# stevenczwu/SAMBLE

Hardware: NVIDIA B200
Metric: clouds/sec SAMBLE seg fwd (N=2048) (higher is better)
Workload: dtype f32

## Files before the change

samble_b200/csrc/knn_tc.cu:

```cuda
#include <cuda_bf16.h>

#include "common.cuh"
#include "tc_common.cuh"

namespace samble {

constexpr int kTcRows = 128;
constexpr int kTcTile = 128;
constexpr int kTcStages = 5;
constexpr int kTcStagesA = 10;
constexpr int kExt = 4096;
constexpr int kTcCap = 120;
constexpr int kTcListLd = 128;
constexpr int kTcListSm = 129;
constexpr int kTcThreads = 192;

static size_t tc_smem_bytes(int nkt, bool pass_b) {
  return (size_t)(pass_b ? 2 : 1) * nkt * 16384 + (size_t)(pass_b ? kTcStages : kTcStagesA) * 16384
         + 3 * kExt  + (pass_b ? (size_t)kTcRows * kTcListSm * 4 : 0) + 1024 + 256;
}

__device__ __forceinline__ float knn_margin(float aa, float bbmax) {
  const float s = sqrtf(aa * bbmax);
  return (3.0517578e-05f + 0.00012207031f) * s + 3.0517578e-05f * (aa + bbmax);
}

__device__ __forceinline__ float knn_margin_coarse(float aa, float bbmax) {
  const float s = sqrtf(aa * bbmax);
  return (0.0078125f + 3.0517578e-05f + 0.00012207031f) * s + 3.0517578e-05f * (aa + bbmax);
}

__device__ __forceinline__ uint32_t knn_pack(float delta, int j) { return (__float_as_uint(delta) & 0xffff0000u) | (uint32_t)j; }
__device__ __forceinline__ float knn_delta_lo(uint32_t w) { return __uint_as_float(w & 0xffff0000u); }
__device__ __forceinline__ float knn_delta_hi(float lo) { return lo * 1.0079f; }

__device__ __forceinline__ void sort64(float (&v)[64]) {
#pragma unroll
  for (int ls = 1; ls <= 6; ++ls) {
#pragma unroll
    for (int lt = ls - 1; lt >= 0; --lt) {
      const int size = 1 << ls, stride = 1 << lt;
#pragma unroll
      for (int t = 0; t < 32; ++t) {
        const int lo = 2 * t - (t & (stride - 1));
        const int hi = lo + stride;
        const bool up = (lo & size) == 0;
        const float a = v[lo], b = v[hi];
        v[lo] = up ? fminf(a, b) : fmaxf(a, b);
        v[hi] = up ? fmaxf(a, b) : fminf(a, b);
      }
    }
  }
}

template <bool PASS_B, int CS, bool PROF = false>
__global__ void __cluster_dims__(CS, 1, 1) __launch_bounds__(kTcThreads, 1)
    knn_tc_kernel(const __grid_constant__ CUtensorMap map_a_hi, const __grid_constant__ CUtensorMap map_a_lo,
                  const __grid_constant__ CUtensorMap map_b_hi, const __grid_constant__ CUtensorMap map_b_lo,
                  const float* __restrict__ anorm, const float* __restrict__ bext, const unsigned* __restrict__ bbmax_bits,
                  int Nq, int Nr, int Cp, int k, float* __restrict__ thr, uint32_t* __restrict__ cand_out,
                  int* __restrict__ cnt_out, int dbg, long long* __restrict__ prof_out) {
  long long* const prof = PROF ? prof_out : nullptr;
  extern __shared__ uint8_t smem_raw[];
  uint8_t* base = tc::smem_align1024(smem_raw);
  const int nkt = (Cp + 63) / 64;
  constexpr int kPlanes = PASS_B ? 2 : 1;
  constexpr int kStages = PASS_B ? kTcStages : kTcStagesA;
  uint8_t* sA = base;
  uint8_t* sB = sA + (size_t)kPlanes * nkt * 16384;
  uint8_t* sAx = sB + (size_t)kStages * 16384;
  uint8_t* sBx = sAx + kExt;
  uint8_t* tail = sBx + 2 * kExt;
  uint32_t* cand = reinterpret_cast<uint32_t*>(tail);
  uint64_t* bars = reinterpret_cast<uint64_t*>(tail + (PASS_B ? kTcRows * kTcListSm * 4 : 0));
  uint64_t* full = bars;
  uint64_t* empty = bars + kStages;
  uint64_t* tfull = bars + 2 * kStages;
  uint64_t* tempty = tfull + 2;
  uint64_t* afull = tempty + 2;
  uint32_t* tmem_slot = reinterpret_cast<uint32_t*>(afull + 1);

  const int tid = threadIdx.x, warp = tid >> 5, lane = tid & 31;
  const int b = blockIdx.y, q0 = blockIdx.x * kTcRows;
  const int ntiles = (Nr + kTcTile - 1) / kTcTile;
  const uint32_t crank = CS > 1 ? tc::cluster_ctarank() : 0u;
  constexpr uint16_t kMask = (uint16_t)((1u << CS) - 1u);

  for (int p = tid; p < 256; p += kTcThreads) {
    const int row = p >> 1, ch = p & 1;
    *reinterpret_cast<uint4*>(sAx + tc::nosw_offset(row, ch, 128)) = ch == 0 ? make_uint4(0x3f803f80u, 0x00003f80u, 0u, 0u) : make_uint4(0u, 0u, 0u, 0u);
  }
  tc::fence_proxy_async();
  if (tid == 0) {
    for (int s = 0; s < kStages; ++s) {
      tc::mbar_init(&full[s], 1);
      tc::mbar_init(&empty[s], CS);
    }
    for (int a = 0; a < 2; ++a) {
      tc::mbar_init(&tfull[a], 1);
      tc::mbar_init(&tempty[a], 128);
    }
    tc::mbar_init(afull, 1);
    tc::mbar_init_fence();
  }
  if (warp == 0) tc::tmem_alloc(tmem_slot, 256);
  tc::tc_fence_before();
  __syncthreads();
  if (CS > 1) tc::cluster_sync();
  tc::tc_fence_after();
  const uint32_t tmem = *tmem_slot;

  if (warp == 5) {
    if (tc::elect_one()) {
      tc::tma_prefetch_desc(&map_a_hi);
      tc::tma_prefetch_desc(&map_b_hi);
      tc::tma_prefetch_desc(&map_b_lo);
      tc::mbar_arrive_expect_tx(afull, (uint32_t)(kPlanes * nkt) * 16384u);
      for (int kt = 0; kt < nkt; ++kt) {
        tc::tma_load_3d(sA + (size_t)kt * 16384, &map_a_hi, afull, kt * 64, q0, b);
        if (PASS_B) tc::tma_load_3d(sA + (size_t)(nkt + kt) * 16384, &map_a_lo, afull, kt * 64, q0, b);
      }
      const float* ext_g = bext + (size_t)b * ntiles * (kExt / 4);
      int s = 0, ph = 0;
      uint32_t seq = 0;
      long long w_empty = 0;
      const long long p_t0 = PROF ? clock64() : 0;
      for (int t = 0; t < ntiles; ++t) {
        for (int g = 0; g < kPlanes * nkt; ++g, ++seq) {
          const int kt = PASS_B ? g >> 1 : g;
          const long long p_t = (PROF && prof) ? clock64() : 0;
          tc::mbar_wait(&empty[s], ph ^ 1);
          if (PROF && prof) w_empty += clock64() - p_t;
          if (g == 0) {
            if (t >= 2) tc::mbar_wait(&tfull[t & 1], ((t - 2) >> 1) & 1);
            tc::mbar_arrive_expect_tx(&full[s], 16384u + kExt);
            tc::bulk_load_1d(sBx + (size_t)(t & 1) * kExt, ext_g + (size_t)t * (kExt / 4), kExt, &full[s]);
          } else {
            tc::mbar_arrive_expect_tx(&full[s], 16384u);
          }
          const CUtensorMap* mp = (PASS_B && (g & 1)) ? &map_b_lo : &map_b_hi;
          if (CS == 1)
            tc::tma_load_3d(sB + (size_t)s * 16384, mp, &full[s], kt * 64, t * kTcTile, b);
          else if (seq % CS == crank)
            tc::tma_load_3d_multicast(sB + (size_t)s * 16384, mp, &full[s], kt * 64, t * kTcTile, b, kMask);
          if (++s == kStages) { s = 0; ph ^= 1; }
        }
      }
      if (PROF && prof) {
        long long* o = prof + 8 * (blockIdx.y * gridDim.x + blockIdx.x);
        o[5] = clock64() - p_t0, o[6] = w_empty;
      }
    }
    __syncwarp();
  } else if (warp == 4) {
    if (tc::elect_one()) {
      const uint32_t idesc = tc::instr_desc(1, kTcRows, kTcTile);
      const uint64_t axd = tc::smem_desc_nosw(tc::smem_u32(sAx), 128);
      long long w_full = 0, w_tempty = 0, w_a = 0, w_issue = 0;
      const long long m_t0 = PROF ? clock64() : 0;
      tc::mbar_wait(afull, 0);
      if (PROF && prof) w_a = clock64() - m_t0;
      int s = 0, ph = 0;
      for (int t = 0; t < ntiles; ++t) {
        const int acc = t & 1;
        long long m_t = (PROF && prof) ? clock64() : 0;
        tc::mbar_wait(&tempty[acc], ((t >> 1) & 1) ^ 1);
        if (PROF && prof) w_tempty += clock64() - m_t;
        tc::tc_fence_after();
        for (int g = 0; g < kPlanes * nkt; ++g) {
          const int kt = PASS_B ? g >> 1 : g;
          m_t = (PROF && prof) ? clock64() : 0;
          tc::mbar_wait(&full[s], ph);
          if (PROF && prof) w_full += clock64() - m_t;
          tc::tc_fence_after();
          const long long i_t = (PROF && prof) ? clock64() : 0;
          const uint64_t ah = tc::smem_desc_sw128(tc::smem_u32(sA + (size_t)kt * 16384));
          const uint64_t al = tc::smem_desc_sw128(tc::smem_u32(sA + (size_t)(nkt + kt) * 16384));
          const uint64_t bd = tc::smem_desc_sw128(tc::smem_u32(sB + (size_t)s * 16384));
          if (dbg & 1) {
          } else if (!PASS_B || (g & 1) == 0) {
#pragma unroll
            for (int k16 = 0; k16 < 4; ++k16) tc::mma_bf16(tmem + acc * kTcTile, ah + 2 * k16, bd + 2 * k16, idesc, (g | k16) != 0);
            if (PASS_B) {
#pragma unroll
              for (int k16 = 0; k16 < 4; ++k16) tc::mma_bf16(tmem + acc * kTcTile, al + 2 * k16, bd + 2 * k16, idesc, 1);
            }
          } else {
#pragma unroll
            for (int k16 = 0; k16 < 4; ++k16) tc::mma_bf16(tmem + acc * kTcTile, ah + 2 * k16, bd + 2 * k16, idesc, 1);
          }
          if (PROF && prof) w_issue += clock64() - i_t;
          if (g == kPlanes * nkt - 1) {
            if (!(dbg & 1)) tc::mma_bf16(tmem + acc * kTcTile, axd, tc::smem_desc_nosw(tc::smem_u32(sBx + (size_t)(t & 1) * kExt), 128), idesc, 1);
          }
          if (CS == 1) tc::mma_commit(&empty[s]);
          else tc::mma_commit_multicast(&empty[s], kMask);
          if (++s == kStages) { s = 0; ph ^= 1; }
        }
        tc::mma_commit(&tfull[acc]);
      }
      if (PROF && prof) {
        long long* o = prof + 8 * (blockIdx.y * gridDim.x + blockIdx.x);
        o[0] = clock64() - m_t0, o[1] = w_full, o[2] = w_tempty, o[3] = w_a, o[7] = w_issue;
      }
    }
    __syncwarp();
  } else {
    const int row = warp * 32 + lane;
    const int q = q0 + row;
    const uint32_t lane_base = (uint32_t)(warp * 32) << 16;
    float gmax[64];
    float my_thr = 0.f;
    const uint32_t lbeg = tc::smem_u32(cand + row * kTcListSm);
    uint32_t lptr = lbeg;
    if (!PASS_B) {
#pragma unroll
      for (int i = 0; i < 64; ++i) gmax[i] = -INFINITY;
    } else {
      my_thr = q < Nq ? thr[(size_t)b * Nq + q] : INFINITY;
    }
    long long w_tfull = 0;
    for (int t = 0; t < ntiles; ++t) {
      const int acc = t & 1;
      const long long e_t = (PROF && prof) ? clock64() : 0;
      tc::mbar_wait(&tfull[acc], (t >> 1) & 1);
      if (PROF && prof) w_tfull += clock64() - e_t;
      tc::tc_fence_after();
      if (!(dbg & 2))
#pragma unroll
      for (int c0 = 0; c0 < kTcTile; c0 += 64) {
        float v[64];
        tc::tmem_ld64(tmem + lane_base + acc * kTcTile + c0, v);
        if (!PASS_B) {
#pragma unroll
          for (int i = 0; i < 64; ++i) gmax[i] = fmaxf(gmax[i], v[i]);
        } else {
          const int jbase = t * kTcTile + c0;
#pragma unroll
          for (int i = 0; i < 64; ++i) {
            const float delta = v[i] - my_thr;
            asm volatile("st.shared.u32 [%0], %1;" ::"r"(lptr), "r"(knn_pack(delta, jbase + i)) : "memory");
            lptr += delta >= 0.f ? 4u : 0u;
            if ((i & 7) == 7) lptr = min(lptr, lbeg + 4u * kTcCap);
          }
        }
      }
      tc::tc_fence_before();
      tc::mbar_arrive(&tempty[acc]);
    }
    if (PROF && prof && tid == 0) prof[8 * (blockIdx.y * gridDim.x + blockIdx.x) + 4] = w_tfull;
    if (!PASS_B) {
      if (q < Nq) {
        sort64(gmax);
        float kth = INFINITY;
#pragma unroll
        for (int i = 32; i < 64; ++i) kth = fminf(kth, i >= 64 - k ? gmax[i] : INFINITY);
        const float aa = anorm[(size_t)b * Nq + q];
        const float bbm = __uint_as_float(bbmax_bits[b]);
        const float e = knn_margin(aa, bbm), ea = knn_margin_coarse(aa, bbm);
        thr[(size_t)b * Nq + q] = fminf(kth - 0.5f * (ea + e), 0.5f * (aa - e));
      }
    } else if (q < Nq) {
      cnt_out[(size_t)b * Nq + q] = (int)(min(lptr, lbeg + 4u * kTcCap) - lbeg) >> 2;
    }
  }

  if (PASS_B) {
    __syncthreads();
    for (int row = warp; row < kTcRows; row += kTcThreads / 32) {
      const int q = q0 + row;
      if (q >= Nq) break;
#pragma unroll
      for (int u = 0; u < 4; ++u)
        cand_out[((size_t)b * Nq + q) * kTcListLd + u * 32 + lane] = cand[row * kTcListSm + u * 32 + lane];
    }
  }
  tc::tc_fence_before();
  __syncthreads();
  if (CS > 1) tc::cluster_sync();
  if (warp == 0) tc::tmem_dealloc(tmem, 256);
}

template <class I>
__device__ __forceinline__ void knn_exact_row(const float* __restrict__ arow, float aa, const float* __restrict__ B_g,
                                              const float* __restrict__ bnorm_g, int Nr, int Cp, int k, int lane,
                                              I* __restrict__ idx_row, float* __restrict__ dist_row, bool ordered) {
  const float4* ar = reinterpret_cast<const float4*>(arow);
  LaneTopK top;
  top.init(lane, k);
  for (int j0 = 0; j0 < Nr; j0 += 128) {
    float acc[4] = {0.f, 0.f, 0.f, 0.f};
    const float4* br[4];
#pragma unroll
    for (int u = 0; u < 4; ++u) br[u] = reinterpret_cast<const float4*>(B_g + (size_t)min(j0 + 32 * u + lane, Nr - 1) * Cp);
#pragma unroll 2
    for (int c4 = 0; c4 < Cp / 4; ++c4) {
      const float4 a4 = __ldg(ar + c4);
#pragma unroll
      for (int u = 0; u < 4; ++u) {
        const float4 b4 = __ldg(br[u] + c4);
        acc[u] = fmaf(a4.x, b4.x, acc[u]);
        acc[u] = fmaf(a4.y, b4.y, acc[u]);
        acc[u] = fmaf(a4.z, b4.z, acc[u]);
        acc[u] = fmaf(a4.w, b4.w, acc[u]);
      }
    }
#pragma unroll
    for (int u = 0; u < 4; ++u) {
      const int j = j0 + 32 * u + lane;
      const bool have = j < Nr;
      const float d2 = __fmaf_rn(-2.f, acc[u], __fadd_rn(aa, __ldg(bnorm_g + min(j, Nr - 1))));
      top.offer(dist_bits(d2), j, have);
    }
  }
  const int pos = ordered ? top.rank() : lane;
  if (top.active) {
    idx_row[pos] = (I)top.i;
    if (dist_row) dist_row[pos] = -sqrtf(__uint_as_float(top.d));
  }
}

template <class I>
__global__ void __launch_bounds__(256) knn_rerank_kernel(const float* __restrict__ an, const float* __restrict__ anorm,
                                                         const float* __restrict__ bn, const float* __restrict__ bnorm,
                                                         const uint32_t* __restrict__ cand,
                                                         const int* __restrict__ cnt_in, int Nq, int Nr, int Cp, int k,
                                                         I* __restrict__ idx_out, float* __restrict__ dist_out,
                                                         int* __restrict__ row_flags) {
  const int warp = threadIdx.x >> 5, lane = threadIdx.x & 31;
  const int b = blockIdx.y, q = blockIdx.x * 8 + warp;
  if (q >= Nq) return;
  const size_t rowi = (size_t)b * Nq + q;
  const int cnt = cnt_in[rowi];
  const float aa = anorm[rowi];
  const float4* ar = reinterpret_cast<const float4*>(an + rowi * Cp);
  const float* B_g = bn + (size_t)b * Nr * Cp;
  const float* bnorm_g = bnorm + (size_t)b * Nr;
  if (cnt >= kTcCap) {
    knn_exact_row<I>(an + rowi * Cp, aa, B_g, bnorm_g, Nr, Cp, k, lane, idx_out + rowi * k, dist_out ? dist_out + rowi * k : nullptr, true);
    return;
  }
  LaneTopK top;
  top.init(lane, k);
  for (int r = 0; r < cnt; r += 32) {
    const int e = r + lane;
    const bool have = e < cnt;
    const int j = have ? (int)(cand[rowi * kTcListLd + e] & 0xffffu) : 0;
    const float4* br = reinterpret_cast<const float4*>(B_g + (size_t)j * Cp);
    float acc = 0.f;
#pragma unroll 4
    for (int c4 = 0; c4 < Cp / 4; ++c4) {
      const float4 a4 = __ldg(ar + c4);
      const float4 b4 = __ldg(br + c4);
      acc = fmaf(a4.x, b4.x, acc);
      acc = fmaf(a4.y, b4.y, acc);
      acc = fmaf(a4.z, b4.z, acc);
      acc = fmaf(a4.w, b4.w, acc);
    }
    const float d2 = __fmaf_rn(-2.f, acc, __fadd_rn(aa, __ldg(bnorm_g + j)));
    const unsigned db = dist_bits(d2);
    if (r == 0 && cnt >= k) {
      top.fill(db, j, have && lane < k);
      top.offer(db, j, have && lane >= k);
    } else {
      top.offer(db, j, have);
    }
  }
  const int rk = top.rank();
  if (top.active) {
    const long long o = (long long)rowi * k + rk;
    idx_out[o] = (I)top.i;
    if (dist_out) dist_out[o] = -sqrtf(__uint_as_float(top.d));
  }
}

template <int NPL, class I>
__device__ __forceinline__ void select_classify(const uint32_t* __restrict__ list, int cnt, int k, float aa, float e,
                                                float thr_row, int lane, I* __restrict__ idx_row,
                                                unsigned short* __restrict__ amb, int& n_in, int& n_amb) {
  constexpr int kN = 32 * NPL;
  uint32_t w[NPL], x[NPL];
#pragma unroll
  for (int u = 0; u < NPL; ++u) {
    const int t = u * 32 + lane;
    w[u] = t < cnt ? __ldg(list + t) : 0u;
    x[u] = ~w[u];
  }
#pragma unroll
  for (int size = 2; size <= kN; size <<= 1) {
#pragma unroll
    for (int stride = size >> 1; stride >= 1; stride >>= 1) {
      if (stride >= 32) {
        const int du = stride >> 5;
#pragma unroll
        for (int u = 0; u < NPL; ++u) {
          if ((u & du) == 0) {
            const bool up = ((u * 32) & size) == 0;
            const uint32_t lo = min(x[u], x[u | du]), hi = max(x[u], x[u | du]);
            x[u] = up ? lo : hi;
            x[u | du] = up ? hi : lo;
          }
        }
      } else {
#pragma unroll
        for (int u = 0; u < NPL; ++u) {
          const uint32_t other = __shfl_xor_sync(kFull, x[u], stride);
          const bool up = ((u * 32 + lane) & size) == 0;
          const bool lower = (lane & stride) == 0;
          x[u] = (lower == up) ? min(x[u], other) : max(x[u], other);
        }
      }
    }
  }
  uint32_t xk = 0xffffffffu, xk1 = 0xffffffffu;
#pragma unroll
  for (int u = 0; u < NPL; ++u) {
    const uint32_t a0 = __shfl_sync(kFull, x[u], (k - 1) & 31);
    const uint32_t a1 = __shfl_sync(kFull, x[u], k & 31);
    if (((k - 1) >> 5) == u) xk = a0;
    if ((k >> 5) == u) xk1 = a1;
  }
  const float dk = knn_delta_lo(~xk);
  const float dk1 = cnt > k ? knn_delta_lo(~xk1) : -INFINITY;
  const float n0 = (0.5f * (aa - e) - thr_row) * 0.999f;
  const bool in_ok = knn_delta_hi(dk1) < n0 || cnt == k;
  const float in_thr = knn_delta_hi(dk1) + e;
  const float out_thr = dk - e;
  const unsigned lt = (1u << lane) - 1u;
#pragma unroll
  for (int u = 0; u < NPL; ++u) {
    const bool have = u * 32 + lane < cnt;
    const float dlo = knn_delta_lo(w[u]), dhi = knn_delta_hi(dlo);
    const int j = (int)(w[u] & 0xffffu);
    const bool is_in = have && in_ok && dlo > in_thr;
    const bool is_out = have && dhi < out_thr && dhi < n0;
    const bool is_amb = have && !is_in && !is_out;
    const unsigned m_in = __ballot_sync(kFull, is_in), m_amb = __ballot_sync(kFull, is_amb);
    if (is_in) idx_row[n_in + __popc(m_in & lt)] = (I)j;
    if (is_amb) amb[n_amb + __popc(m_amb & lt)] = (unsigned short)j;
    n_in += __popc(m_in);
    n_amb += __popc(m_amb);
  }
}

constexpr int kSelBatch = 4;
constexpr int kSelRowLd = 132;

template <class I>
__global__ void __launch_bounds__(256, 5) knn_select_kernel(const float* __restrict__ an, const float* __restrict__ anorm,
                                                         const float* __restrict__ bn, const float* __restrict__ bnorm,
                                                         const unsigned* __restrict__ bbmax_bits,
                                                         const uint32_t* __restrict__ cand,
                                                         const float* __restrict__ thr_in, const int* __restrict__ cnt_in,
                                                         int Nq, int Nr, int Cp, int k, I* __restrict__ idx_out,
                                                         int* __restrict__ row_flags) {
  __shared__ unsigned short amb[8][128];
  __shared__ __align__(16) float s_arow[8][128];
  __shared__ __align__(16) float s_rows[8][kSelBatch * kSelRowLd];
  __shared__ unsigned long long s_keys[8][128];
  const int warp = threadIdx.x >> 5, lane = threadIdx.x & 31;
  const int b = blockIdx.y, q = blockIdx.x * 8 + warp;
  if (q >= Nq) return;
  const size_t rowi = (size_t)b * Nq + q;
  const int cnt = cnt_in[rowi];
  const float aa = anorm[rowi];
  if (cnt >= kTcCap) {
    knn_exact_row<I>(an + rowi * Cp, aa, bn + (size_t)b * Nr * Cp, bnorm + (size_t)b * Nr, Nr, Cp, k, lane, idx_out + rowi * k, nullptr, false);
    return;
  }
  const float e = knn_margin(aa, __uint_as_float(bbmax_bits[b])) * 1.001f;
  int n_in = 0, n_amb = 0;
  const uint32_t* list = cand + rowi * kTcListLd;
  const float thr_row = __ldg(thr_in + rowi);
  if (cnt <= 32)
    select_classify<1, I>(list, cnt, k, aa, e, thr_row, lane, idx_out + rowi * k, amb[warp], n_in, n_amb);
  else if (cnt <= 64)
    select_classify<2, I>(list, cnt, k, aa, e, thr_row, lane, idx_out + rowi * k, amb[warp], n_in, n_amb);
  else
    select_classify<4, I>(list, cnt, k, aa, e, thr_row, lane, idx_out + rowi * k, amb[warp], n_in, n_amb);
  const int need = k - n_in;
  if (need <= 0) return;
  if (n_amb < need) {
    __syncwarp();
    knn_exact_row<I>(an + rowi * Cp, aa, bn + (size_t)b * Nr * Cp, bnorm + (size_t)b * Nr, Nr, Cp, k, lane, idx_out + rowi * k, nullptr, false);
    return;
  }
  __syncwarp();
  const int nch = Cp >> 2;
  const float4* ar = reinterpret_cast<const float4*>(an + rowi * Cp);
  const float* B_g = bn + (size_t)b * Nr * Cp;
  const float* bnorm_g = bnorm + (size_t)b * Nr;
  if (lane < nch) reinterpret_cast<float4*>(s_arow[warp])[lane] = __ldg(ar + lane);
  for (int r = 0; r < n_amb; r += kSelBatch) {
    const int nb = min(kSelBatch, n_amb - r);
    float4 tmp[kSelBatch];
#pragma unroll
    for (int u = 0; u < kSelBatch; ++u)
      if (u < nb && lane < nch) tmp[u] = __ldg(reinterpret_cast<const float4*>(B_g + (size_t)amb[warp][r + u] * Cp) + lane);
#pragma unroll
    for (int u = 0; u < kSelBatch; ++u)
      if (u < nb && lane < nch) reinterpret_cast<float4*>(s_rows[warp] + u * kSelRowLd)[lane] = tmp[u];
    __syncwarp();
    if (lane < nb) {
      const int j = (int)amb[warp][r + lane];
      const float4* br = reinterpret_cast<const float4*>(s_rows[warp] + lane * kSelRowLd);
      const float4* aq = reinterpret_cast<const float4*>(s_arow[warp]);
      float acc = 0.f;
#pragma unroll 4
      for (int c4 = 0; c4 < nch; ++c4) {
        const float4 a4 = aq[c4];
        const float4 b4 = br[c4];
        acc = fmaf(a4.x, b4.x, acc);
        acc = fmaf(a4.y, b4.y, acc);
        acc = fmaf(a4.z, b4.z, acc);
        acc = fmaf(a4.w, b4.w, acc);
      }
      const float d2 = __fmaf_rn(-2.f, acc, __fadd_rn(aa, __ldg(bnorm_g + j)));
      s_keys[warp][r + lane] = ((unsigned long long)dist_bits(d2) << 32) | (unsigned)j;
    }
    __syncwarp();
  }
  for (int t = lane; t < n_amb; t += 32) {
    const unsigned long long mine = s_keys[warp][t];
    int rank = 0;
    for (int u = 0; u < n_amb; ++u) rank += s_keys[warp][u] < mine ? 1 : 0;
    if (rank < need) idx_out[rowi * k + n_in + rank] = (I)(unsigned)(mine & 0xffffffffu);
  }
}

int g_knn_tc_debug = 0;
int g_knn_cluster = -1;
long long* g_knn_prof = nullptr;

size_t knn_tc_ext_floats(int B, int Nr);
bool knn_tc_eligible(int Nq, int Nr, int C, int k) {
  const int Cp = (int)align_up(C, 32);
  return C >= 4 && Cp <= 128 && k <= 32 && Nr <= 65535 && Nr >= k;
}

size_t knn_tc_workspace_bytes(int B, int Nq, int Nr) {
  return align_up((size_t)B * Nq * kTcListLd * sizeof(uint32_t), 256) + align_up((size_t)B * Nq * sizeof(int), 256) +
         align_up(knn_tc_ext_floats(B, Nr) * sizeof(float), 256);
}
size_t knn_tc_ext_floats(int B, int Nr) { return (size_t)B * ceil_div(Nr, kTcTile) * (kExt / 4); }

template <class I>
int launch_knn_tc(const float* an, const float* anorm, const float* bn, const float* bnorm, const __nv_bfloat16* a_hi,
                  const __nv_bfloat16* a_lo, const __nv_bfloat16* b_hi, const __nv_bfloat16* b_lo, const float* bext,
                  const unsigned* bbmax, int B, int Nq, int Nr, int Cp, int k, float* thr, uint32_t* cand, int* cnt, bool ordered,
                  I* idx, float* dist, int* row_flags, cudaStream_t st) {
  const int nkb = (Cp + 63) / 64;
  alignas(64) CUtensorMap map_a, map_al, map_b, map_bl;
  if (int e = make_tile_map(&map_a, a_hi, Cp, Cp, Nq, B, kTcRows, 2)) return e;
  if (int e = make_tile_map(&map_al, a_lo, Cp, Cp, Nq, B, kTcRows, 2)) return e;
  if (int e = make_tile_map(&map_b, b_hi, Cp, Cp, Nr, B, kTcTile, 2)) return e;
  if (int e = make_tile_map(&map_bl, b_lo, Cp, Cp, Nr, B, kTcTile, 2)) return e;
  dim3 grid(ceil_div(Nq, kTcRows), B);
  const int cs = g_knn_cluster > 0 ? g_knn_cluster : 1;
  {
    size_t smem = tc_smem_bytes(nkb, false);
    auto kern = cs == 2 ? knn_tc_kernel<false, 2> : (cs == 4 ? knn_tc_kernel<false, 4> : (g_knn_prof ? knn_tc_kernel<false, 1, true> : knn_tc_kernel<false, 1>));
    if (cudaFuncSetAttribute(kern, cudaFuncAttributeMaxDynamicSharedMemorySize, (int)smem) != cudaSuccess)
      return check_launch("knn_tc pass A smem attribute");
    SAMBLE_PRE(st);
    kern<<<grid, kTcThreads, smem, st>>>(map_a, map_al, map_b, map_bl, anorm, bext, bbmax, Nq, Nr, Cp, k, thr, cand, cnt, g_knn_tc_debug, g_knn_prof);
    SAMBLE_LAUNCHED("knn_tc_threshold_kernel");
  }
  {
    size_t smem = tc_smem_bytes(nkb, true);
    auto kern = cs == 2 ? knn_tc_kernel<true, 2> : (cs == 4 ? knn_tc_kernel<true, 4> : (g_knn_prof ? knn_tc_kernel<true, 1, true> : knn_tc_kernel<true, 1>));
    if (cudaFuncSetAttribute(kern, cudaFuncAttributeMaxDynamicSharedMemorySize, (int)smem) != cudaSuccess)
      return check_launch("knn_tc pass B smem attribute");
    SAMBLE_PRE(st);
    kern<<<grid, kTcThreads, smem, st>>>(map_a, map_al, map_b, map_bl, anorm, bext, bbmax, Nq, Nr, Cp, k, thr, cand, cnt, g_knn_tc_debug, g_knn_prof);
    SAMBLE_LAUNCHED("knn_tc_collect_kernel");
  }
  SAMBLE_PRE(st);
  if (ordered) {
    knn_rerank_kernel<I><<<dim3(ceil_div(Nq, 8), B), 256, 0, st>>>(an, anorm, bn, bnorm, cand, cnt, Nq, Nr, Cp, k, idx, dist, row_flags);
    SAMBLE_LAUNCHED("knn_rerank_kernel");
  } else {
    knn_select_kernel<I><<<dim3(ceil_div(Nq, 8), B), 256, 0, st>>>(an, anorm, bn, bnorm, bbmax, cand, thr, cnt, Nq, Nr, Cp, k, idx, row_flags);
    SAMBLE_LAUNCHED("knn_select_kernel");
  }
  return SAMBLE_OK;
}

template int launch_knn_tc<int>(const float*, const float*, const float*, const float*, const __nv_bfloat16*, const __nv_bfloat16*,
                                const __nv_bfloat16*, const __nv_bfloat16*, const float*, const unsigned*, int, int, int, int, int,
                                float*, uint32_t*, int*, bool, int*, float*, int*, cudaStream_t);
template int launch_knn_tc<long long>(const float*, const float*, const float*, const float*, const __nv_bfloat16*,
                                      const __nv_bfloat16*, const __nv_bfloat16*, const __nv_bfloat16*, const float*, const unsigned*,
                                      int, int, int, int, int, float*, uint32_t*, int*, bool, long long*, float*, int*,
                                      cudaStream_t);

}

extern "C" void samble_set_knn_probe(long long* cycles) { samble::g_knn_prof = cycles; }
extern "C" void samble_set_knn_debug(int bits) { samble::g_knn_tc_debug = bits & 0xff; samble::g_knn_cluster = (bits >> 8) ? (bits >> 8) : -1; }
```

Before: 4959.

## Pair two query tiles per CTA in kNN tensor-core kernels to reuse B tiles

Adds a QT=2 variant of the kNN tensor-core threshold and collect kernels. One CTA holds two 128-row query tiles and issues MMAs for both against each streamed reference tile, using twice the TMEM columns and 8 epilogue warps. It is selected when the number of CTAs would exceed the SM count, which halves reference-tile TMA traffic and pipeline overhead per query. In exchange the pass-B candidate lists go straight to global memory instead of being staged in shared memory, and there are fewer CTAs and fewer pass-A pipeline stages.

Measured after the change: 5064 (median of 6 runs). 1.02x the previous value.

```diff
diff --git a/samble_b200/csrc/knn_tc.cu b/samble_b200/csrc/knn_tc.cu
--- a/samble_b200/csrc/knn_tc.cu
+++ b/samble_b200/csrc/knn_tc.cu
@@ -1,4 +1,6 @@
 #include <cuda_bf16.h>
+
+#include <atomic>
 
 #include "common.cuh"
 #include "tc_common.cuh"
@@ -9,16 +11,23 @@
 constexpr int kTcTile = 128;
 constexpr int kTcStages = 5;
 constexpr int kTcStagesA = 10;
+constexpr int kTcStagesA2 = 8;
 constexpr int kExt = 4096;
 constexpr int kTcCap = 120;
 constexpr int kTcListLd = 128;
 constexpr int kTcListSm = 129;
-constexpr int kTcThreads = 192;
-
-static size_t tc_smem_bytes(int nkt, bool pass_b) {
-  return (size_t)(pass_b ? 2 : 1) * nkt * 16384 + (size_t)(pass_b ? kTcStages : kTcStagesA) * 16384
-         + 3 * kExt  + (pass_b ? (size_t)kTcRows * kTcListSm * 4 : 0) + 1024 + 256;
-}
+
+constexpr int tc_threads(int qt) { return 32 * (4 * qt + 2); }
+constexpr int tc_stages(bool pass_b, int qt) { return pass_b ? kTcStages : (qt == 2 ? kTcStagesA2 : kTcStagesA); }
+constexpr bool tc_smem_lists(bool pass_b, int qt) { return pass_b && qt == 1; }
+
+constexpr size_t tc_smem_bytes(int nkt, bool pass_b, int qt) {
+  return (size_t)qt * (pass_b ? 2 : 1) * nkt * 16384 + (size_t)tc_stages(pass_b, qt) * 16384
+         + 3 * kExt  + (tc_smem_lists(pass_b, qt) ? (size_t)kTcRows * kTcListSm * 4 : 0) + 1024 + 256;
+}
+static_assert(tc_smem_bytes(2, false, 1) <= 227 * 1024 && tc_smem_bytes(2, true, 1) <= 227 * 1024 &&
+                  tc_smem_bytes(2, false, 2) <= 227 * 1024 && tc_smem_bytes(2, true, 2) <= 227 * 1024,
+              "knn_tc shared memory exceeds the 227 KB a block can have");
 
 __device__ __forceinline__ float knn_margin(float aa, float bbmax) {
   const float s = sqrtf(aa * bbmax);
@@ -53,26 +62,29 @@
   }
 }
 
-template <bool PASS_B, int CS, bool PROF = false>
-__global__ void __cluster_dims__(CS, 1, 1) __launch_bounds__(kTcThreads, 1)
+template <bool PASS_B, int QT, int CS, bool PROF = false>
+__global__ void __cluster_dims__(CS, 1, 1) __launch_bounds__(tc_threads(QT), 1)
     knn_tc_kernel(const __grid_constant__ CUtensorMap map_a_hi, const __grid_constant__ CUtensorMap map_a_lo,
                   const __grid_constant__ CUtensorMap map_b_hi, const __grid_constant__ CUtensorMap map_b_lo,
                   const float* __restrict__ anorm, const float* __restrict__ bext, const unsigned* __restrict__ bbmax_bits,
                   int Nq, int Nr, int Cp, int k, float* __restrict__ thr, uint32_t* __restrict__ cand_out,
                   int* __restrict__ cnt_out, int dbg, long long* __restrict__ prof_out) {
+  static_assert(QT == 1 || (QT == 2 && CS == 1 && !PROF), "paired query tiles run without clusters and cycle probes");
+  constexpr int kThreads = tc_threads(QT);
+  constexpr bool kSmemLists = tc_smem_lists(PASS_B, QT);
   long long* const prof = PROF ? prof_out : nullptr;
   extern __shared__ uint8_t smem_raw[];
   uint8_t* base = tc::smem_align1024(smem_raw);
   const int nkt = (Cp + 63) / 64;
   constexpr int kPlanes = PASS_B ? 2 : 1;
-  constexpr int kStages = PASS_B ? kTcStages : kTcStagesA;
+  constexpr int kStages = tc_stages(PASS_B, QT);
   uint8_t* sA = base;
-  uint8_t* sB = sA + (size_t)kPlanes * nkt * 16384;
+  uint8_t* sB = sA + (size_t)QT * kPlanes * nkt * 16384;
   uint8_t* sAx = sB + (size_t)kStages * 16384;
   uint8_t* sBx = sAx + kExt;
   uint8_t* tail = sBx + 2 * kExt;
   uint32_t* cand = reinterpret_cast<uint32_t*>(tail);
-  uint64_t* bars = reinterpret_cast<uint64_t*>(tail + (PASS_B ? kTcRows * kTcListSm * 4 : 0));
+  uint64_t* bars = reinterpret_cast<uint64_t*>(tail + (kSmemLists ? kTcRows * kTcListSm * 4 : 0));
   uint64_t* full = bars;
   uint64_t* empty = bars + kStages;
   uint64_t* tfull = bars + 2 * kStages;
@@ -81,12 +93,13 @@
   uint32_t* tmem_slot = reinterpret_cast<uint32_t*>(afull + 1);
 
   const int tid = threadIdx.x, warp = tid >> 5, lane = tid & 31;
-  const int b = blockIdx.y, q0 = blockIdx.x * kTcRows;
+  const int b = blockIdx.y, q0 = blockIdx.x * (QT * kTcRows);
   const int ntiles = (Nr + kTcTile - 1) / kTcTile;
+  const int nlive = QT > 1 && q0 + kTcRows >= Nq ? 1 : QT;
   const uint32_t crank = CS > 1 ? tc::cluster_ctarank() : 0u;
   constexpr uint16_t kMask = (uint16_t)((1u << CS) - 1u);
 
-  for (int p = tid; p < 256; p += kTcThreads) {
+  for (int p = tid; p < 256; p += kThreads) {
     const int row = p >> 1, ch = p & 1;
     *reinterpret_cast<uint4*>(sAx + tc::nosw_offset(row, ch, 128)) = ch == 0 ? make_uint4(0x3f803f80u, 0x00003f80u, 0u, 0u) : make_uint4(0u, 0u, 0u, 0u);
   }
@@ -98,27 +111,30 @@
     }
     for (int a = 0; a < 2; ++a) {
       tc::mbar_init(&tfull[a], 1);
-      tc::mbar_init(&tempty[a], 128);
+      tc::mbar_init(&tempty[a], QT * 128);
     }
     tc::mbar_init(afull, 1);
     tc::mbar_init_fence();
   }
-  if (warp == 0) tc::tmem_alloc(tmem_slot, 256);
+  if (warp == 0) tc::tmem_alloc(tmem_slot, 256 * QT);
   tc::tc_fence_before();
   __syncthreads();
   if (CS > 1) tc::cluster_sync();
   tc::tc_fence_after();
   const uint32_t tmem = *tmem_slot;
 
-  if (warp == 5) {
+  if (warp == 4 * QT + 1) {
     if (tc::elect_one()) {
       tc::tma_prefetch_desc(&map_a_hi);
       tc::tma_prefetch_desc(&map_b_hi);
       tc::tma_prefetch_desc(&map_b_lo);
-      tc::mbar_arrive_expect_tx(afull, (uint32_t)(kPlanes * nkt) * 16384u);
-      for (int kt = 0; kt < nkt; ++kt) {
-        tc::tma_load_3d(sA + (size_t)kt * 16384, &map_a_hi, afull, kt * 64, q0, b);
-        if (PASS_B) tc::tma_load_3d(sA + (size_t)(nkt + kt) * 16384, &map_a_lo, afull, kt * 64, q0, b);
+      tc::mbar_arrive_expect_tx(afull, (uint32_t)(nlive * kPlanes * nkt) * 16384u);
+      for (int u = 0; u < nlive; ++u) {
+        uint8_t* sAu = sA + (size_t)u * kPlanes * nkt * 16384;
+        for (int kt = 0; kt < nkt; ++kt) {
+          tc::tma_load_3d(sAu + (size_t)kt * 16384, &map_a_hi, afull, kt * 64, q0 + u * kTcRows, b);
+          if (PASS_B) tc::tma_load_3d(sAu + (size_t)(nkt + kt) * 16384, &map_a_lo, afull, kt * 64, q0 + u * kTcRows, b);
+        }
       }
       const float* ext_g = bext + (size_t)b * ntiles * (kExt / 4);
       int s = 0, ph = 0;
@@ -152,7 +168,7 @@
       }
     }
     __syncwarp();
-  } else if (warp == 4) {
+  } else if (warp == 4 * QT) {
     if (tc::elect_one()) {
       const uint32_t idesc = tc::instr_desc(1, kTcRows, kTcTile);
       const uint64_t axd = tc::smem_desc_nosw(tc::smem_u32(sAx), 128);
@@ -174,25 +190,26 @@
           if (PROF && prof) w_full += clock64() - m_t;
           tc::tc_fence_after();
           const long long i_t = (PROF && prof) ? clock64() : 0;
-          const uint64_t ah = tc::smem_desc_sw128(tc::smem_u32(sA + (size_t)kt * 16384));
-          const uint64_t al = tc::smem_desc_sw128(tc::smem_u32(sA + (size_t)(nkt + kt) * 16384));
           const uint64_t bd = tc::smem_desc_sw128(tc::smem_u32(sB + (size_t)s * 16384));
-          if (dbg & 1) {
-          } else if (!PASS_B || (g & 1) == 0) {
-#pragma unroll
-            for (int k16 = 0; k16 < 4; ++k16) tc::mma_bf16(tmem + acc * kTcTile, ah + 2 * k16, bd + 2 * k16, idesc, (g | k16) != 0);
-            if (PASS_B) {
-#pragma unroll
-              for (int k16 = 0; k16 < 4; ++k16) tc::mma_bf16(tmem + acc * kTcTile, al + 2 * k16, bd + 2 * k16, idesc, 1);
+          for (int u = 0; u < nlive && !(dbg & 1); ++u) {
+            const uint32_t d = tmem + (uint32_t)((acc * QT + u) * kTcTile);
+            const uint8_t* sAu = sA + (size_t)u * kPlanes * nkt * 16384;
+            const uint64_t ah = tc::smem_desc_sw128(tc::smem_u32(sAu + (size_t)kt * 16384));
+            const uint64_t al = tc::smem_desc_sw128(tc::smem_u32(sAu + (size_t)(nkt + kt) * 16384));
+            if (!PASS_B || (g & 1) == 0) {
+#pragma unroll
+              for (int k16 = 0; k16 < 4; ++k16) tc::mma_bf16(d, ah + 2 * k16, bd + 2 * k16, idesc, (g | k16) != 0);
+              if (PASS_B) {
+#pragma unroll
+                for (int k16 = 0; k16 < 4; ++k16) tc::mma_bf16(d, al + 2 * k16, bd + 2 * k16, idesc, 1);
+              }
+            } else {
+#pragma unroll
+              for (int k16 = 0; k16 < 4; ++k16) tc::mma_bf16(d, ah + 2 * k16, bd + 2 * k16, idesc, 1);
             }
-          } else {
-#pragma unroll
-            for (int k16 = 0; k16 < 4; ++k16) tc::mma_bf16(tmem + acc * kTcTile, ah + 2 * k16, bd + 2 * k16, idesc, 1);
+            if (g == kPlanes * nkt - 1) tc::mma_bf16(d, axd, tc::smem_desc_nosw(tc::smem_u32(sBx + (size_t)(t & 1) * kExt), 128), idesc, 1);
           }
           if (PROF && prof) w_issue += clock64() - i_t;
-          if (g == kPlanes * nkt - 1) {
-            if (!(dbg & 1)) tc::mma_bf16(tmem + acc * kTcTile, axd, tc::smem_desc_nosw(tc::smem_u32(sBx + (size_t)(t & 1) * kExt), 128), idesc, 1);
-          }
           if (CS == 1) tc::mma_commit(&empty[s]);
           else tc::mma_commit_multicast(&empty[s], kMask);
           if (++s == kStages) { s = 0; ph ^= 1; }
@@ -206,13 +223,17 @@
     }
     __syncwarp();
   } else {
-    const int row = warp * 32 + lane;
-    const int q = q0 + row;
-    const uint32_t lane_base = (uint32_t)(warp * 32) << 16;
+    const int u = warp >> 2;
+    const int row = (warp & 3) * 32 + lane;
+    const int q = q0 + u * kTcRows + row;
+    const bool live = u < nlive;
+    const uint32_t lane_base = (uint32_t)((warp & 3) * 32) << 16;
     float gmax[64];
     float my_thr = 0.f;
     const uint32_t lbeg = tc::smem_u32(cand + row * kTcListSm);
     uint32_t lptr = lbeg;
+    uint32_t* const glist = cand_out + ((size_t)b * Nq + q) * kTcListLd;
+    int gcnt = 0;
     if (!PASS_B) {
 #pragma unroll
       for (int i = 0; i < 64; ++i) gmax[i] = -INFINITY;
@@ -226,16 +247,16 @@
       tc::mbar_wait(&tfull[acc], (t >> 1) & 1);
       if (PROF && prof) w_tfull += clock64() - e_t;
       tc::tc_fence_after();
-      if (!(dbg & 2))
+      if (live && !(dbg & 2))
 #pragma unroll
       for (int c0 = 0; c0 < kTcTile; c0 += 64) {
         float v[64];
-        tc::tmem_ld64(tmem + lane_base + acc * kTcTile + c0, v);
+        tc::tmem_ld64(tmem + lane_base + (uint32_t)((acc * QT + u) * kTcTile + c0), v);
+        const int jbase = t * kTcTile + c0;
         if (!PASS_B) {
 #pragma unroll
           for (int i = 0; i < 64; ++i) gmax[i] = fmaxf(gmax[i], v[i]);
-        } else {
-          const int jbase = t * kTcTile + c0;
+        } else if (kSmemLists) {
 #pragma unroll
           for (int i = 0; i < 64; ++i) {
             const float delta = v[i] - my_thr;
@@ -243,6 +264,14 @@
             lptr += delta >= 0.f ? 4u : 0u;
             if ((i & 7) == 7) lptr = min(lptr, lbeg + 4u * kTcCap);
           }
+        } else {
+#pragma unroll
+          for (int i = 0; i < 64; ++i) {
+            const float delta = v[i] - my_thr;
+            if (delta >= 0.f) glist[gcnt] = knn_pack(delta, jbase + i);
+            gcnt += delta >= 0.f ? 1 : 0;
+            if ((i & 7) == 7) gcnt = min(gcnt, kTcCap);
+          }
         }
       }
       tc::tc_fence_before();
@@ -261,13 +290,13 @@
         thr[(size_t)b * Nq + q] = fminf(kth - 0.5f * (ea + e), 0.5f * (aa - e));
       }
     } else if (q < Nq) {
-      cnt_out[(size_t)b * Nq + q] = (int)(min(lptr, lbeg + 4u * kTcCap) - lbeg) >> 2;
-    }
-  }
-
-  if (PASS_B) {
+      cnt_out[(size_t)b * Nq + q] = kSmemLists ? (int)(min(lptr, lbeg + 4u * kTcCap) - lbeg) >> 2 : min(gcnt, kTcCap);
+    }
+  }
+
+  if (kSmemLists) {
     __syncthreads();
-    for (int row = warp; row < kTcRows; row += kTcThreads / 32) {
+    for (int row = warp; row < kTcRows; row += kThreads / 32) {
       const int q = q0 + row;
       if (q >= Nq) break;
 #pragma unroll
@@ -278,7 +307,7 @@
   tc::tc_fence_before();
   __syncthreads();
   if (CS > 1) tc::cluster_sync();
-  if (warp == 0) tc::tmem_dealloc(tmem, 256);
+  if (warp == 0) tc::tmem_dealloc(tmem, 256 * QT);
 }
 
 template <class I>
@@ -544,6 +573,24 @@
 }
 size_t knn_tc_ext_floats(int B, int Nr) { return (size_t)B * ceil_div(Nr, kTcTile) * (kExt / 4); }
 
+static cudaError_t current_sm_count(int* n) {
+  static std::atomic<int> cache[64];
+  int dev = 0;
+  if (cudaError_t e = cudaGetDevice(&dev)) return e;
+  if (dev < 64 && (*n = cache[dev].load(std::memory_order_relaxed)) > 0) return cudaSuccess;
+  if (cudaError_t e = cudaDeviceGetAttribute(n, cudaDevAttrMultiProcessorCount, dev)) return e;
+  if (dev < 64) cache[dev].store(*n, std::memory_order_relaxed);
+  return cudaSuccess;
+}
+
+template <bool PASS_B>
+static decltype(&knn_tc_kernel<PASS_B, 1, 1>) pick_knn_tc(bool pair, int cs) {
+  if (pair) return knn_tc_kernel<PASS_B, 2, 1>;
+  if (cs == 2) return knn_tc_kernel<PASS_B, 1, 2>;
+  if (cs == 4) return knn_tc_kernel<PASS_B, 1, 4>;
+  return g_knn_prof ? knn_tc_kernel<PASS_B, 1, 1, true> : knn_tc_kernel<PASS_B, 1, 1>;
+}
+
 template <class I>
 int launch_knn_tc(const float* an, const float* anorm, const float* bn, const float* bnorm, const __nv_bfloat16* a_hi,
                   const __nv_bfloat16* a_lo, const __nv_bfloat16* b_hi, const __nv_bfloat16* b_lo, const float* bext,
@@ -555,25 +602,32 @@
   if (int e = make_tile_map(&map_al, a_lo, Cp, Cp, Nq, B, kTcRows, 2)) return e;
   if (int e = make_tile_map(&map_b, b_hi, Cp, Cp, Nr, B, kTcTile, 2)) return e;
   if (int e = make_tile_map(&map_bl, b_lo, Cp, Cp, Nr, B, kTcTile, 2)) return e;
-  dim3 grid(ceil_div(Nq, kTcRows), B);
   const int cs = g_knn_cluster > 0 ? g_knn_cluster : 1;
+  int sms = 0;
+  if (cudaError_t e = current_sm_count(&sms)) {
+    set_error("knn_tc SM count: %s", cudaGetErrorString(e));
+    return SAMBLE_E_CUDA;
+  }
+  const bool pair = cs == 1 && !g_knn_prof && (long long)B * ceil_div(Nq, kTcRows) > sms;
+  const int qt = pair ? 2 : 1;
+  const dim3 grid(ceil_div(Nq, qt * kTcRows), B);
   {
-    size_t smem = tc_smem_bytes(nkb, false);
-    auto kern = cs == 2 ? knn_tc_kernel<false, 2> : (cs == 4 ? knn_tc_kernel<false, 4> : (g_knn_prof ? knn_tc_kernel<false, 1, true> : knn_tc_kernel<false, 1>));
+    size_t smem = tc_smem_bytes(nkb, false, qt);
+    auto kern = pick_knn_tc<false>(pair, cs);
     if (cudaFuncSetAttribute(kern, cudaFuncAttributeMaxDynamicSharedMemorySize, (int)smem) != cudaSuccess)
       return check_launch("knn_tc pass A smem attribute");
     SAMBLE_PRE(st);
-    kern<<<grid, kTcThreads, smem, st>>>(map_a, map_al, map_b, map_bl, anorm, bext, bbmax, Nq, Nr, Cp, k, thr, cand, cnt, g_knn_tc_debug, g_knn_prof);
-    SAMBLE_LAUNCHED("knn_tc_threshold_kernel");
+    kern<<<grid, tc_threads(qt), smem, st>>>(map_a, map_al, map_b, map_bl, anorm, bext, bbmax, Nq, Nr, Cp, k, thr, cand, cnt, g_knn_tc_debug, g_knn_prof);
+    SAMBLE_LAUNCHED(pair ? "knn_tc_threshold_pair_kernel" : "knn_tc_threshold_kernel");
   }
   {
-    size_t smem = tc_smem_bytes(nkb, true);
-    auto kern = cs == 2 ? knn_tc_kernel<true, 2> : (cs == 4 ? knn_tc_kernel<true, 4> : (g_knn_prof ? knn_tc_kernel<true, 1, true> : knn_tc_kernel<true, 1>));
+    size_t smem = tc_smem_bytes(nkb, true, qt);
+    auto kern = pick_knn_tc<true>(pair, cs);
     if (cudaFuncSetAttribute(kern, cudaFuncAttributeMaxDynamicSharedMemorySize, (int)smem) != cudaSuccess)
       return check_launch("knn_tc pass B smem attribute");
     SAMBLE_PRE(st);
-    kern<<<grid, kTcThreads, smem, st>>>(map_a, map_al, map_b, map_bl, anorm, bext, bbmax, Nq, Nr, Cp, k, thr, cand, cnt, g_knn_tc_debug, g_knn_prof);
-    SAMBLE_LAUNCHED("knn_tc_collect_kernel");
+    kern<<<grid, tc_threads(qt), smem, st>>>(map_a, map_al, map_b, map_bl, anorm, bext, bbmax, Nq, Nr, Cp, k, thr, cand, cnt, g_knn_tc_debug, g_knn_prof);
+    SAMBLE_LAUNCHED(pair ? "knn_tc_collect_pair_kernel" : "knn_tc_collect_kernel");
   }
   SAMBLE_PRE(st);
   if (ordered) {
```
